# ibejarano/Pynama

Hardware: AMD Instinct MI355X
Metric: assembled element-DOFs/sec + CG iterations/sec, 10M-DOF Poisson, 1/2/4/8 MI355X (higher is better)
Workload: dtype f64

## Files before the change

include/pynama_hip.h:

```cpp
#ifndef PYNAMA_HIP_H
#define PYNAMA_HIP_H

#include <stdint.h>

#ifdef __cplusplus
extern "C" {
#endif

typedef struct pyn_ctx pyn_ctx;

enum {
  PYN_OK = 0,
  PYN_EINVAL = -1,
  PYN_EHIP = -2,
  PYN_ENCCL = -3,
  PYN_ENOTCONV = -4,
  PYN_ENOGPU = -5
};

enum { PYN_Q_FULL = 0, PYN_Q_RED = 1, PYN_Q_NODAL = 2 };

enum {
  PYN_FORM_LAPLACE = 0,
  PYN_FORM_MASS_NODAL = 1,
// ... 81 lines not shown
int pyn_vec_maxpy(pyn_ctx* ctx, int y, int x, int m, const int* ids, const double* w);
int pyn_ts_step_finish(pyn_ctx* ctx, int x, int m, const int* ids, const double* hb, const double* hd, double atol, double rtol,
                       double* wnorm);

int pyn_nodeset_create(pyn_ctx* ctx, int64_t n, const int32_t* nodes, int* set_id);
int pyn_nodeset_destroy(pyn_ctx* ctx, int set_id);
enum {
  PYN_FIELD_TG2D_VEL = 0, PYN_FIELD_TG2D_VORT = 1,
  PYN_FIELD_TG3D_VEL = 2, PYN_FIELD_TG3D_VORT = 3, PYN_FIELD_TG3D_CONV = 4, PYN_FIELD_TG3D_DIFF = 5,
  PYN_FIELD_SEN2D_VEL = 6, PYN_FIELD_SEN2D_VORT = 7, PYN_FIELD_SEN2D_CONV = 8, PYN_FIELD_SEN2D_DIFF = 9,
  PYN_FIELD_COUNT = 10
};
#define PYN_FIELD_MAX_PARAMS 4
int pyn_field_info(int field, int* dim, int* bs, int* nparams);
int pyn_field_eval(pyn_ctx* ctx, int field, const double* params, int nparams, int set_id, int vec_id);
int pyn_vec_set_nodes(pyn_ctx* ctx, int vec_id, int set_id, const double* values, int nvalues, const uint8_t* dofs);

int pyn_assemble_kle(pyn_ctx* ctx, double alpha_d, double alpha_w, int K, int Krhs, int Rw, int Rd,
                     int variant);
int pyn_assemble_kle_noslip(pyn_ctx* ctx, double alpha_d, double alpha_w, const int* mat_ids);
int pyn_assemble_scalar(pyn_ctx* ctx, int form, int A, int Arhs, int variant);
int pyn_elem_local(pyn_ctx* ctx, int form, double alpha_d, double alpha_w, const double* corners,
                   double* out0, double* out1, double* out2);

int pyn_assemble_operator(pyn_ctx* ctx, int rule, int nterms, const int32_t* terms, const double* coef, int mat_id);
int pyn_elem_operator_local(pyn_ctx* ctx, int rule, int br, int bc, int nterms, const int32_t* terms,
                            const double* coef, const double* corners, double* out);

int pyn_spmv(pyn_ctx* ctx, int mat_id, int x_vec, int y_vec);
int pyn_product_last(pyn_ctx* ctx, int64_t* info);
int pyn_product_choose(int br, int bc, int npat, int maxw, int64_t nnzb, int64_t n_owned, int rhs_compact, int solver, int image,
                       int sell_image, int block_sell, int no_csrlb, int no_sell, double bcsr_min_avg, int bcsr_lanes, int bcsr_unroll,
                       int* kind, int* W, int* lanes, int* unroll);
int pyn_assemble_last(pyn_ctx* ctx, int64_t* info);
int pyn_assemble_choose(const int64_t* request, const int64_t* facts, const int64_t* knobs, int64_t* out);
int pyn_assemble_choose_layout(char* buf, int len);
enum { PYN_MATFREE_OFF = 0, PYN_MATFREE_LAPLACE = 1, PYN_MATFREE_KLE = 2, PYN_MATFREE_KLE_GENERAL = 3,
       PYN_MATFREE_KLE_NGL3_GENERAL = 4 };
int pyn_matfree_set(pyn_ctx* ctx, int op, double alpha_d, double alpha_w);
int pyn_matfree_apply(pyn_ctx* ctx, int op, int x_vec, int y_vec);
typedef struct pyn_solve_opts {
  int method;
  int pc;
  int norm_type;
  int maxit;
  int restart;
  int fixed_iters;
  int profile;
  int cg_variant;
  int gmres_orthog;
  int matfree;
  double rtol, atol, dtol;
} pyn_solve_opts;
typedef struct pyn_solve_info {
  int iters;
  int reason;
  double rnorm;
  double rnorm0;
  double true_resid;
  double solve_ms;
  double spmv_ms;
  int spmv_launches;
  double reduce_ms;
  double halo_ms;
} pyn_solve_info;
int pyn_solve(pyn_ctx* ctx, int mat_id, int b_vec, int x_vec, const pyn_solve_opts* opts,
// ... 35 lines not shown
```

pynama_amd/_lib.py:

```python
from __future__ import annotations

import ctypes as C
import os
import subprocess
import sys

import numpy as np

_HERE = os.path.dirname(os.path.abspath(__file__))
LIB_PATH = os.environ.get("PYNAMA_LIB_PATH") or os.path.join(_HERE, "libpynama_hip.so")
CSRC = os.path.join(_HERE, "csrc")

Q_FULL, Q_RED, Q_NODAL = 0, 1, 2
FORM_LAPLACE, FORM_MASS_NODAL, FORM_MASS_FULL, FORM_KLE, FORM_OPERATOR = 0, 1, 2, 3, 4
KSP_CG, KSP_GMRES = 0, 1
MATFREE_OFF, MATFREE_LAPLACE, MATFREE_KLE, MATFREE_KLE_GENERAL, MATFREE_KLE_NGL3_GENERAL = 0, 1, 2, 3, 4
PC_NONE, PC_JACOBI, PC_MG = 0, 1, 2
MG_MAX_LEVELS = 16
TS_MAX_STAGES = 8
NORM_PRECONDITIONED, NORM_UNPRECONDITIONED, NORM_NATURAL = 0, 1, 2
T_SYMBOLIC, T_ASSEMBLE, T_SPMV, T_SOLVE = 0, 1, 2, 3
(FIELD_TG2D_VEL, FIELD_TG2D_VORT, FIELD_TG3D_VEL, FIELD_TG3D_VORT, FIELD_TG3D_CONV, FIELD_TG3D_DIFF,
 FIELD_SEN2D_VEL, FIELD_SEN2D_VORT, FIELD_SEN2D_CONV, FIELD_SEN2D_DIFF) = range(10)
FIELD_COUNT, FIELD_MAX_PARAMS = 10, 4
# ... 66 lines not shown
    "pyn_mat_get_values": [_P, _I, _pf64],
    "pyn_mat_get_diagonal": [_P, _I, _I],
    "pyn_mat_axpy": [_P, _I, _D, _I],
    "pyn_mat_row_scale": [_P, _I, _I],
    "pyn_vec_create": [_P, _I, C.POINTER(_I)],
    "pyn_vec_destroy": [_P, _I],
    "pyn_vec_set_host": [_P, _I, _pf64],
    "pyn_vec_set_local_host": [_P, _I, _pf64],
    "pyn_vec_get_host": [_P, _I, _pf64],
    "pyn_vec_fill": [_P, _I, _D],
    "pyn_vec_scatter_host": [_P, _I, _L, _pi32, _pf64, _I],
    "pyn_vec_axpby": [_P, _I, _D, _I, _D, _I],
    "pyn_vec_pointwise_mult": [_P, _I, _I, _I],
    "pyn_vec_reciprocal": [_P, _I],
    "pyn_vec_vtensv": [_P, _I, _I],
    "pyn_vec_dot": [_P, _I, _I, C.POINTER(_D)],
    "pyn_vec_norm": [_P, _I, _I, C.POINTER(_D)],
    "pyn_vec_maxpy": [_P, _I, _I, _I, _pi32, _pf64],
    "pyn_ts_step_finish": [_P, _I, _I, _pi32, _pf64, _P, _D, _D, C.POINTER(_D)],
    "pyn_nodeset_create": [_P, _L, _P, C.POINTER(_I)],
    "pyn_nodeset_destroy": [_P, _I],
    "pyn_field_info": [_I, C.POINTER(_I), C.POINTER(_I), C.POINTER(_I)],
    "pyn_field_eval": [_P, _I, _pf64, _I, _I, _I],
    "pyn_vec_set_nodes": [_P, _I, _I, _pf64, _I, _P],
    "pyn_assemble_kle": [_P, _D, _D, _I, _I, _I, _I, _I],
    "pyn_assemble_kle_noslip": [_P, _D, _D, C.POINTER(_I)],
    "pyn_assemble_scalar": [_P, _I, _I, _I, _I],
    "pyn_elem_local": [_P, _I, _D, _D, _pf64, _P, _P, _P],
    "pyn_assemble_operator": [_P, _I, _I, _pi32, _pf64, _I],
    "pyn_elem_operator_local": [_P, _I, _I, _I, _I, _pi32, _pf64, _pf64, _pf64],
    "pyn_spmv": [_P, _I, _I, _I],
    "pyn_product_last": [_P, _pi64],
    "pyn_product_choose": [_I] * 4 + [_L, _L] + [_I] * 7 + [_D, _I, _I] + [C.POINTER(_I)] * 4,
    "pyn_assemble_last": [_P, _pi64],
    "pyn_assemble_choose": [_pi64, _pi64, _pi64, _pi64],
    "pyn_assemble_choose_layout": [C.c_char_p, _I],
    "pyn_matfree_apply": [_P, _I, _I, _I],
    "pyn_matfree_set": [_P, _I, _D, _D],
    "pyn_solve": [_P, _I, _I, _I, C.POINTER(SolveOpts), C.POINTER(SolveInfo)],
    "pyn_direct_max_rows": [],
    "pyn_solve_direct": [_P, _I, _I, _I, C.POINTER(SolveInfo)],
    "pyn_direct_band_info": [_P, _I, C.POINTER(_L), C.POINTER(_L), C.POINTER(_L)],
    "pyn_solve_direct_band": [_P, _I, _I, _I, _L, C.POINTER(SolveInfo)],
    "pyn_mg_setup": [_P, _I, C.POINTER(MgOpts)],
    "pyn_mg_info": [_P, _I, C.POINTER(_I), _pi64, _pf64, C.POINTER(_D), C.POINTER(_I)],
    "pyn_mg_apply": [_P, _I, _I, _I],
    "pyn_mg_level_get": [_P, _I, _I, _pf64],
    "pyn_ibm_set": [_P, _I, _I, _L, _pf64, _pf64, _pf64, _pf64],
    "pyn_ibm_interp": [_P, _I, _pf64],
    "pyn_ibm_spread": [_P, _pf64, _I],
    "pyn_ibm_correct": [_P, _I, _pf64, _pf64],
    "pyn_ibm_matrix_get": [_P, _pf64],
    "pyn_ibm_info": [_P, _pi64],
    "pyn_ibm_clear": [_P],
    "pyn_timers_get": [_P, _pf64, _I],
}

_lib = None


def build_library(force=False):
    if force:
        subprocess.check_call(["make", "-C", CSRC, "clean"])
    subprocess.check_call(["make", "-C", CSRC, "-j4"])
    return LIB_PATH

# ... 46 lines not shown

def ho_tables_1d(ngl):
    n = int(ngl)
    if n < 2:
        raise PynamaHipError(f"ho_tables_1d: ngl {n} out of range")
    t = dict(xl=np.zeros(n), wl=np.zeros(n), Dl=np.zeros((n, n)), xr=np.zeros(n - 1), wr=np.zeros(n - 1),
             Br=np.zeros((n - 1, n)), Gr=np.zeros((n - 1, n)))
    _check(load_library().pyn_ho_tables_1d(n, *(t[k] for k in ("xl", "wl", "Dl", "xr", "wr", "Br", "Gr"))))
    return t


def ho_local_lattice(ngl, dim):
    loc = np.zeros((int(ngl) ** int(dim), int(dim)), np.int32)
    _check(load_library().pyn_ho_local_lattice(int(ngl), int(dim), loc))
    return loc


def field_info(field):
    d, b, n = _I(0), _I(0), _I(0)
    _check(load_library().pyn_field_info(int(field), C.byref(d), C.byref(b), C.byref(n)))
    return d.value, b.value, n.value


def product_choose(br, bc, npat, maxw, nnzb, n_owned, rhs_compact=False, solver=False, image=False, sell_image=False,
                   block_sell=False, no_csrlb=False, no_sell=False, bcsr_min_avg=None, bcsr_lanes=None, bcsr_unroll=None):
    out = [_I(0) for _ in range(4)]
    _check(load_library().pyn_product_choose(
        int(br), int(bc), int(npat), int(maxw), int(nnzb), int(n_owned), int(rhs_compact), int(solver), int(image), int(sell_image),
        int(block_sell), int(no_csrlb), int(no_sell), -1.0 if bcsr_min_avg is None else float(bcsr_min_avg),
        -1 if bcsr_lanes is None else int(bcsr_lanes), -1 if bcsr_unroll is None else int(bcsr_unroll), *(C.byref(o) for o in out)))
    return tuple(o.value for o in out)


ASSEMBLY_KINDS = ("none", "generic", "p1", "patch", "lattice", "march", "kle_lattice", "rowrun")
AK_NONE, AK_GENERIC, AK_P1, AK_PATCH, AK_LATTICE, AK_MARCH, AK_KLE_LATTICE, AK_ROWRUN = range(8)
_ASM_LAST_KEYS = ("kind", "shape", "k_closed", "rw_closed", "generic", "krhs_completed", "dinv", "count")


def assemble_choose_layout():
    buf = C.create_string_buffer(4096)
    _check(load_library().pyn_assemble_choose_layout(buf, len(buf)))
    return {part.split(":")[0]: tuple(n for n in part.split(":")[1].split(",") if n) for part in buf.value.decode().split(";")}


def assemble_choose(request, facts, knobs=None):
    layout = assemble_choose_layout()
    given = {"request": dict({"variant": 1}, **request), "facts": dict(facts), "knobs": dict(knobs or {})}
    arrays = {}
    for part, names in layout.items():
        unknown = set(given[part]) - set(names)
        if unknown:
            raise PynamaHipError(f"assemble_choose: unknown {part} {sorted(unknown)}")
        arrays[part] = np.array([int(given[part].get(n, -1 if part == "knobs" else 0)) for n in names], np.int64)
    out = np.zeros(8, np.int64)
    _check(load_library().pyn_assemble_choose(arrays["request"], arrays["facts"], arrays["knobs"], out))
    return dict({k: int(v) for k, v in zip(_ASM_LAST_KEYS[:7], out)}, rowrun_candidate=int(out[7]))


class _stdout_to_stderr:

    def __enter__(self):
        sys.stdout.flush()
        self._saved = os.dup(1)
        os.dup2(2, 1)

    def __exit__(self, *exc):
# ... 489 lines not shown
```

pynama_amd/csrc/pyn_internal.h:

```cpp
#pragma once
#include <hip/hip_runtime.h>
#include <rccl/rccl.h>

#include <algorithm>
#include <atomic>
#include <cstdint>
#include <cstdio>
#include <functional>
#include <map>
#include <memory>
#include <string>
#include <type_traits>
#include <utility>
#include <vector>

#include "../../include/pynama_hip.h"

void pyn_set_error(const char* fmt, ...);

#define PYN_HIP(call)                                                                         \
  do {                                                                                        \
    hipError_t e_ = (call);                                                                   \
    if (e_ != hipSuccess) {                                                                   \
      pyn_set_error("%s:%d %s -> %s", __FILE__, __LINE__, #call, hipGetErrorString(e_));      \
// ... 68 lines not shown
  T* get() const { return p_; }
  operator T*() const { return p_; }
};
template <typename T>
using DevBuf = Buf<T, false>;
template <typename T>
using PinBuf = Buf<T, true>;

struct DevTmp : DevBuf<unsigned char> {
  template <typename T>
  T* as() const {
    return reinterpret_cast<T*>(get());
  }
};

template <typename T>
inline int dev_upload(DevBuf<T>& dst, const T* src, size_t n, hipStream_t s) {
  PYN_HIP(dst.alloc(n));
  if (n && src) PYN_HIP(hipMemcpyAsync(dst.get(), src, n * sizeof(T), hipMemcpyHostToDevice, s));
  return PYN_OK;
}

struct QuadTab {
  int ngp = 0;
  DevBuf<double> w;
  DevBuf<double> H;
  DevBuf<double> Hrs;
  DevBuf<double> HrsCoo;
  double wsum = 0.0;
  bool const_grad = false;
};

enum ProductKind { PK_NONE = 0, PK_RAW = 1, PK_SELL = 2, PK_SELLP = 3, PK_SELLB_X = 4, PK_SELLB_D = 5, PK_CSRL = 6, PK_CSRLB = 7, PK_BCSR = 8 };
struct ProductPlan {
  ProductKind kind = PK_NONE;
  int W = 0;
  int lg = 0, unroll = 0;
  size_t lds = 0;
  int wg_cap = -1;
  int max_grid = INT32_MAX;
};

struct MgHier;
struct IbmState;
struct MgHierDelete { void operator()(MgHier* h) const; };
struct IbmStateDelete { void operator()(IbmState* s) const; };

struct DMat {
  int br = 0, bc = 0;
  DevBuf<double> val;
  DevBuf<double> sell_val;
  bool sell_valid = false;
  ProductPlan plan;
  DevBuf<double> dinv;
  bool dinv_valid = false;
  DevBuf<double> lu;
  DevBuf<int> lu_piv;
  int64_t lu_n = 0;
  bool lu_valid = false;
  DevBuf<double> band;
  DevBuf<int> band_perm;
  int64_t band_n = 0, band_kl = 0, band_ku = 0;
  bool band_valid = false;
  std::unique_ptr<MgHier, MgHierDelete> mg;
  bool mg_valid = false;
  int64_t rhs_clean = -2;
  bool rhs_compact = false;
  int64_t c_stamp = -1;
  int64_t c_nr = 0, c_nnzb = 0;
  DevBuf<int32_t> c_crow;
  DevBuf<int32_t> c_rsel;
  DevBuf<int32_t> c_cptr;
  bool live = false;
// ... 397 lines not shown
```

pynama_amd/csrc/pyn_sell.hip:

```cpp
#include <hipcub/hipcub.hpp>

#include "pyn_internal.h"

namespace {

constexpr int PAT_MAX = 256;
constexpr int PAT_W = 32;

constexpr int SH = 64;

__global__ void sell_width_kernel(const int32_t* __restrict__ rowptr, int64_t n_rows, int br, int bc, int64_t n_slices,
                                  int* __restrict__ w) {
  for (int64_t s = (int64_t)blockIdx.x * blockDim.x + threadIdx.x; s < n_slices; s += (int64_t)gridDim.x * blockDim.x) {
    int64_t r0 = s * SH, r1 = r0 + SH < n_rows ? r0 + SH : n_rows;
    int m = 0;
    for (int64_t r = r0; r < r1; ++r) {
      const int64_t i = r / br;
      m = max(m, (rowptr[i + 1] - rowptr[i]) * bc);
    }
    w[s] = m;
  }
}

template <bool WITH_COLS>
// ... 188 lines not shown
  for (int64_t r = (int64_t)blockIdx.x * blockDim.x + threadIdx.x; r < n_rows; r += (int64_t)gridDim.x * blockDim.x) {
    const unsigned long long x = h[r];
    int l = 0, hgh = nu;
    while (l < hgh) {
      int m = (l + hgh) >> 1;
      if (uniq[m] < x)
        l = m + 1;
      else
        hgh = m;
    }
    pid[r] = l;
    rep[l] = (int32_t)r;
  }
}

__global__ void pat_table_kernel(const int32_t* __restrict__ rowptr, const int32_t* __restrict__ colidx,
                                 const int32_t* __restrict__ rep, int nu, int32_t* __restrict__ tab, int32_t* __restrict__ tlen) {
  const int p = blockIdx.x;
  if (p >= nu) return;
  const int r = rep[p];
  const int lo = rowptr[r], len = rowptr[r + 1] - lo;
  if (threadIdx.x == 0) tlen[p] = len;
  for (int k = threadIdx.x; k < PAT_W; k += blockDim.x) tab[p * PAT_W + k] = k < len ? colidx[lo + k] - r : 0;
}

__global__ void pat_verify_kernel(const int32_t* __restrict__ rowptr, const int32_t* __restrict__ colidx, int64_t n_rows,
                                  const int32_t* __restrict__ pid, const int32_t* __restrict__ tab,
                                  const int32_t* __restrict__ tlen, int* __restrict__ bad) {
  for (int64_t r = (int64_t)blockIdx.x * blockDim.x + threadIdx.x; r < n_rows; r += (int64_t)gridDim.x * blockDim.x) {
    const int lo = rowptr[r], len = rowptr[r + 1] - lo;
    const int p = pid[r];
    bool ok = len == tlen[p];
    for (int k = 0; ok && k < len; ++k) ok = colidx[lo + k] == (int32_t)r + tab[p * PAT_W + k];
    if (!ok) *bad = 1;
  }
}

template <bool DOT>
__global__ void __launch_bounds__(256) sellp_spmv_kernel(const int64_t* __restrict__ sptr, const int* __restrict__ sw,
                                                         const int32_t* __restrict__ pid, const int32_t* __restrict__ tab,
                                                         int npat, const double* __restrict__ sval,
                                                         const double* __restrict__ x, double* __restrict__ y, int64_t n_rows,
                                                         int64_t n_slices, const int* __restrict__ flag,
                                                         double* __restrict__ part, int64_t s_begin, int part_off, int64_t hole_begin, int64_t hole_len) {
  extern __shared__ int32_t ltab[];
  __shared__ double smd[4];
  if (flag && flag[0]) return;
  for (int i = threadIdx.x; i < (npat + 1) * PAT_W; i += 256) ltab[i] = i < npat * PAT_W ? tab[i] : 0;
  __syncthreads();
  const int lane = threadIdx.x & 63;
  const int64_t w0 = ((int64_t)blockIdx.x * blockDim.x + threadIdx.x) >> 6;
  const int64_t nw = ((int64_t)gridDim.x * blockDim.x) >> 6;
  double dot = 0.0;
  for (int64_t sq = s_begin + w0; sq < n_slices; sq += nw) {
    const int64_t s = sq >= hole_begin ? sq + hole_len : sq;
    const int64_t row = s * SH + lane;
    const int wd = sw[s];
    const double* __restrict__ v = sval + sptr[s] + lane;
    const int32_t* __restrict__ t = ltab + (row < n_rows ? pid[row] : npat) * PAT_W;
    const int64_t rb = row < n_rows ? row : 0;
    double a0 = 0.0, a1 = 0.0, a2 = 0.0, a3 = 0.0;
    int k = 0;
    for (; k + 4 <= wd; k += 4) {
      const double v0 = v[(k + 0) * SH], v1 = v[(k + 1) * SH], v2 = v[(k + 2) * SH], v3 = v[(k + 3) * SH];
      a0 = fma(v0, x[rb + t[k + 0]], a0);
      a1 = fma(v1, x[rb + t[k + 1]], a1);
      a2 = fma(v2, x[rb + t[k + 2]], a2);
      a3 = fma(v3, x[rb + t[k + 3]], a3);
    }
    for (; k < wd; ++k) a0 = fma(v[k * SH], x[rb + t[k]], a0);
    const double acc = (a0 + a1) + (a2 + a3);
    if (row < n_rows) {
      y[row] = acc;
      if (DOT) dot += acc * x[row];
    }
  }
  if (DOT) {
    dot = wsum64(dot);
    if (lane == 0) smd[threadIdx.x >> 6] = dot;
    __syncthreads();
    if (threadIdx.x == 0) part[part_off + blockIdx.x] = smd[0] + smd[1] + smd[2] + smd[3];
  }
}

template <typename T_>
__device__ __forceinline__ T_ ld_stream(const T_* p) {
  return __builtin_nontemporal_load(p);
}

constexpr int CSRL_WAVES = 4;
template <int W, bool DOT>
__global__ void __launch_bounds__(64 * CSRL_WAVES) csrl_spmv_kernel(const int32_t* __restrict__ rowptr, const int32_t* __restrict__ pid,
                                                                    const int32_t* __restrict__ tab, int npat, const double* __restrict__ val,
                                                                    const double* __restrict__ x, double* __restrict__ y, int64_t n_rows,
                                                                    int64_t n_slices, const int* __restrict__ flag, double* __restrict__ part,
                                                                    int64_t s_begin, int part_off, int64_t hole_begin, int64_t hole_len) {
  extern __shared__ double csrl_lds[];
  __shared__ double smd[CSRL_WAVES];
  if (flag && flag[0]) return;
  int32_t* ltab = reinterpret_cast<int32_t*>(csrl_lds + CSRL_WAVES * 64 * W);
  for (int i = threadIdx.x; i < (npat + 1) * PAT_W; i += 64 * CSRL_WAVES) ltab[i] = i < npat * PAT_W ? tab[i] : 0;
  __syncthreads();
  const int lane = threadIdx.x & 63, wv = threadIdx.x >> 6;
  double* __restrict__ buf = csrl_lds + wv * 64 * W;
  const int64_t w0 = (int64_t)blockIdx.x * CSRL_WAVES + wv;
  const int64_t nw = (int64_t)gridDim.x * CSRL_WAVES;
  double dot = 0.0;
  int nrp0 = 0, nrp1 = 0;
  {
    const int64_t sq = s_begin + w0;
    if (sq < n_slices) {
      const int64_t r = (sq >= hole_begin ? sq + hole_len : sq) * SH + lane;
      nrp0 = rowptr[r < n_rows ? r : n_rows];
      nrp1 = rowptr[r < n_rows ? r + 1 : n_rows];
    }
  }
  for (int64_t sq = s_begin + w0; sq < n_slices; sq += nw) {
    const int64_t s = sq >= hole_begin ? sq + hole_len : sq;
    const int64_t row = s * SH + lane;
    const bool live = row < n_rows;
    const int rp0 = nrp0, rp1 = nrp1;
    if (sq + nw < n_slices) {
      const int64_t r = ((sq + nw) >= hole_begin ? sq + nw + hole_len : sq + nw) * SH + lane;
      nrp0 = rowptr[r < n_rows ? r : n_rows];
      nrp1 = rowptr[r < n_rows ? r + 1 : n_rows];
    }
    const int base = __builtin_amdgcn_readfirstlane(rp0);
    const int total = __builtin_amdgcn_readlane(rp1, 63) - base;
    const int off = rp0 - base, len = rp1 - rp0;
    const double* __restrict__ v = val + base;
    double vr[W];
#pragma unroll
    for (int j = 0; j < W; ++j) vr[j] = (64 * j + lane < total) ? ld_stream(v + 64 * j + lane) : 0.0;
    const int32_t* __restrict__ t = ltab + (live ? pid[row] : npat) * PAT_W;
    const int64_t rb = live ? row : 0;
    double xg[W];
#pragma unroll
    for (int k = 0; k < W; ++k) xg[k] = x[rb + (k < len ? t[k] : 0)];
#pragma unroll
    for (int j = 0; j < W; ++j) buf[64 * j + lane] = vr[j];
    __builtin_amdgcn_fence(__ATOMIC_RELEASE, "wavefront");
    __builtin_amdgcn_wave_barrier();
    __builtin_amdgcn_fence(__ATOMIC_ACQUIRE, "wavefront");
    double a0 = 0.0, a1 = 0.0;
#pragma unroll
    for (int k = 0; k + 1 < W; k += 2) {
      a0 = fma(k < len ? buf[off + k] : 0.0, xg[k], a0);
      a1 = fma(k + 1 < len ? buf[off + k + 1] : 0.0, xg[k + 1], a1);
    }
    if (W & 1) a0 = fma(W - 1 < len ? buf[off + W - 1] : 0.0, xg[W - 1], a0);
    const double acc = a0 + a1;
    if (live) {
      y[row] = acc;
      if (DOT) dot += acc * x[row];
    }
    __builtin_amdgcn_fence(__ATOMIC_RELEASE, "wavefront");
    __builtin_amdgcn_wave_barrier();
  }
  if (DOT) {
    dot = wsum64(dot);
    if (lane == 0) smd[wv] = dot;
    __syncthreads();
    if (threadIdx.x == 0) {
      double sm = 0.0;
      for (int i = 0; i < CSRL_WAVES; ++i) sm += smd[i];
      part[part_off + blockIdx.x] = sm;
    }
  }
}

constexpr int CSRLB_WAVES = 2;
template <int W, int BR, int BC, bool GL, bool DOT>
__global__ void __launch_bounds__(64 * CSRLB_WAVES) csrlb_spmv_kernel(const int32_t* __restrict__ rowptr, const int32_t* __restrict__ pid,
                                                                      const int32_t* __restrict__ tab, int npat, const double* __restrict__ val,
                                                                      const double* __restrict__ x, double* __restrict__ y, int64_t n_rows,
                                                                      int64_t n_slices, const int* __restrict__ flag, double* __restrict__ part,
                                                                      int64_t s_begin, int part_off, int64_t hole_begin, int64_t hole_len) {
  extern __shared__ double csrl_lds[];
  __shared__ double smd[CSRLB_WAVES];
  if (flag && flag[0]) return;
  int32_t* ltab = reinterpret_cast<int32_t*>(csrl_lds + CSRLB_WAVES * 64 * W);
  for (int i = threadIdx.x; i < (npat + 1) * PAT_W; i += 64 * CSRLB_WAVES) ltab[i] = i < npat * PAT_W ? tab[i] : 0;
  __syncthreads();
  const int lane = threadIdx.x & 63, wv = threadIdx.x >> 6;
  double* __restrict__ buf = csrl_lds + wv * 64 * W;
  const int64_t w0 = (int64_t)blockIdx.x * CSRLB_WAVES + wv;
  const int64_t nw = (int64_t)gridDim.x * CSRLB_WAVES;
  const int64_t n_nodes = n_rows / BR;
  double dot = 0.0;
  for (int64_t sq = s_begin + w0; sq < n_slices; sq += nw) {
// ... 258 lines not shown
  if (DOT) block_partial(dot, part);
}

}

namespace {
__device__ __forceinline__ int lat_axis_class(int ngl, int c, int N) {
  if (ngl == 2) return c == 0 ? 0 : (c == N - 1 ? 2 : 1);
  if (c & 1) return 3;
  return c == 0 ? 0 : (c == N - 1 ? 2 : 1);
}
__global__ void pat_lattice_pid_kernel(int ngl, int dim, int NX, int NY, int NZ, int64_t n_rows, int32_t* __restrict__ pid) {
  const int64_t i = (int64_t)blockIdx.x * blockDim.x + threadIdx.x;
  if (i >= n_rows) return;
  const int ncls = ngl == 2 ? 3 : 4;
  const int x = (int)(i % NX), y = (int)((i / NX) % NY), z = (int)(i / ((int64_t)NX * NY));
  int id = lat_axis_class(ngl, y, NY) * ncls + lat_axis_class(ngl, x, NX);
  if (dim == 3) id += lat_axis_class(ngl, z, NZ) * ncls * ncls;
  pid[i] = id;
}
__global__ void pat_verify_sample_kernel(const int32_t* __restrict__ rowptr, const int32_t* __restrict__ colidx, int64_t n_rows, int64_t stride,
                                         const int32_t* __restrict__ pid, const int32_t* __restrict__ tab, const int32_t* __restrict__ tlen,
                                         int* __restrict__ bad) {
  const int64_t t = (int64_t)blockIdx.x * blockDim.x + threadIdx.x;
  int64_t r = t * stride;
  if (r >= n_rows) {
    if (r - stride >= n_rows || t == 0) return;
    r = n_rows - 1;
  }
  const int lo = rowptr[r], len = rowptr[r + 1] - lo;
  const int p = pid[r];
  bool ok = len == tlen[p];
  for (int k = 0; ok && k < len; ++k) ok = colidx[lo + k] == (int32_t)r + tab[p * PAT_W + k];
  if (!ok) *bad = 1;
}
}

static int lattice_pattern_dictionary(pyn_ctx* c, bool* done) {
  *done = false;
  if (getenv("PYNAMA_NO_LATTICE_PATTERNS")) return PYN_OK;
  const BoxLattice& B = c->box;
  if (!(c->lat.valid || c->ho3.valid) || (B.ngl == 3 && B.dim == 3) || c->n_ghost != 0 || !B.natural()) return PYN_OK;
  const int ngl = B.ngl, dim = B.dim, NX = B.NX, NY = B.ny(), NZ = B.nz();
  const int ncls = ngl == 2 ? 3 : 4;
  const int npat = dim == 3 ? ncls * ncls * ncls : ncls * ncls;
  auto axis_offs = [&](int cls, int* out) {
    int lo, hi;
    if (ngl == 2) {
      lo = cls == 0 ? 0 : -1;
      hi = cls == 2 ? 0 : 1;
    } else if (cls == 3) {
      lo = -1;
      hi = 1;
    } else {
      lo = cls == 0 ? 0 : -2;
      hi = cls == 2 ? 0 : 2;
    }
    int n = 0;
    for (int d = lo; d <= hi; ++d) out[n++] = d;
    return n;
  };
  std::vector<int32_t> tab((size_t)PAT_MAX * PAT_W, 0), tlen((size_t)PAT_MAX, 0);
  for (int p = 0; p < npat; ++p) {
    const int cx = p % ncls, cy = (p / ncls) % ncls, cz = p / (ncls * ncls);
    int ox[5], oy[5], oz[5] = {0, 0, 0, 0, 0};
    const int nxo = axis_offs(cx, ox), nyo = axis_offs(cy, oy), nzo = dim == 3 ? axis_offs(cz, oz) : 1;
// ... 73 lines not shown
  PYN_HIP(hipMemsetAsync(ptab, 0, (size_t)PAT_MAX * PAT_W * sizeof(int32_t), s));
  pat_assign_kernel<<<grid, 256, 0, s>>>(h, n, hu, (int)nu, pid, t_rep.as<int32_t>());
  pat_table_kernel<<<(int)nu, 64, 0, s>>>(c->d_rowptr, c->d_colidx, t_rep.as<int32_t>(), (int)nu, ptab, t_len.as<int32_t>());
  pat_verify_kernel<<<grid, 256, 0, s>>>(c->d_rowptr, c->d_colidx, n, pid, ptab, t_len.as<int32_t>(), t_bad.as<int>());
  int hbad = 0;
  PYN_HIP(hipMemcpyAsync(&hbad, t_bad.get(), sizeof(int), hipMemcpyDeviceToHost, s));
  PYN_HIP(hipStreamSynchronize(s));
  if (hbad != 0) return PYN_OK;
  c->sell_pid = std::move(pid);
  c->sell_tab = std::move(ptab);
  c->sell_npat = (int)nu;
  return PYN_OK;
}

__global__ void slice_ghost_flag_kernel(const int32_t* __restrict__ rowptr, const int32_t* __restrict__ colidx, int64_t n_owned,
                                        int br, int64_t ns, int* __restrict__ flags) {
  for (int64_t s = (int64_t)blockIdx.x * blockDim.x + threadIdx.x; s < ns; s += (int64_t)gridDim.x * blockDim.x) {
    const int64_t r0 = s * SH, r1 = std::min<int64_t>(r0 + SH, n_owned * br) - 1;
    int f = 0;
    for (int64_t i = r0 / br; i <= r1 / br; ++i) f |= colidx[rowptr[i + 1] - 1] >= n_owned;
    flags[s] = f;
  }
}

struct ProductFacts {
  int br, bc, npat, maxw;
  int64_t nnzb, n_owned;
  bool rhs_compact, solver, image;
};
struct ProductKnobs {
  bool sell_image, block_sell, no_csrlb, no_sell;
  double bcsr_min_avg;
  int bcsr_lanes, bcsr_unroll, bcsr_wgs, csrlb_wgs, csr_wgs, max_grid;
};
static int env_int(const char* name) {
  const char* e = getenv(name);
  return e ? std::max(0, atoi(e)) : -1;
}
static ProductKnobs read_knobs() {
  const char* avg = getenv("PYNAMA_BCSR_MIN_AVG");
  return {getenv("PYNAMA_SELL_IMAGE") != nullptr, getenv("PYNAMA_BLOCK_SELL") != nullptr, getenv("PYNAMA_NO_CSRLB") != nullptr,
          getenv("PYNAMA_NO_SELL") != nullptr, avg ? atof(avg) : 128.0, env_int("PYNAMA_BCSR_LANES"), env_int("PYNAMA_BCSR_UNROLL"),
          env_int("PYNAMA_BCSR_WGS_PER_CU"), env_int("PYNAMA_CSRLB_WGS_PER_CU"), env_int("PYNAMA_CSR_SPMV_WGS_PER_CU"),
          env_int("PYNAMA_SPMV_MAX_GRID")};
}

static bool sell_shape(int bc) { return bc == 1 || bc == 2 || bc == 3 || bc == 6; }
static bool bcsr_shape(int br, int bc) {
  return (br == bc && (br == 1 || br == 2 || br == 3)) || (bc == 1 && (br == 2 || br == 3)) || (br == 1 && (bc == 2 || bc == 3)) ||
         (br == 3 && bc == 2) || (br == 2 && bc == 3) || (br == 6 && bc == 3) || (br == 3 && bc == 6);
}
static bool raw_only(const ProductFacts& f, const ProductKnobs& k) { return !f.rhs_compact && (k.no_sell || !sell_shape(f.bc)); }

static ProductPlan product_choose(const ProductFacts& f, const ProductKnobs& k, bool* keep_image) {
  auto pick = [&](ProductPlan p, bool keep) { *keep_image = keep; return p; };
  const double avg = (double)f.nnzb * f.bc / (double)std::max<int64_t>(1, f.n_owned);
  auto bcsr = [&](bool keep) {
    const int g = k.bcsr_lanes, lg = g >= 0 ? (g >= 64 ? 6 : g >= 32 ? 5 : g >= 16 ? 4 : 3) : (avg >= 56.0 ? 4 : 3);
    const int u = k.bcsr_unroll >= 0 ? k.bcsr_unroll : (avg >= 24.0 ? 8 : 4);
    return pick({PK_BCSR, 0, lg, (u == 2 || u == 3 || u == 8) ? u : 4}, keep);
  };
  const bool scalar = f.br == 1 && f.bc == 1;
  if (f.rhs_compact) return bcsr_shape(f.br, f.bc) ? bcsr(true) : pick({}, true);
  if (raw_only(f, k)) return pick({PK_RAW}, true);
  if (scalar && f.npat > 0 && f.maxw <= PAT_W && !k.sell_image) return pick({PK_CSRL, f.maxw <= 27 ? 27 : 32}, false);
  if (f.br == 2 && f.bc == 2 && f.npat > 0 && f.maxw <= 50 && !k.block_sell && !k.no_csrlb)
    return pick({PK_CSRLB, f.maxw <= 18 ? 18 : (f.maxw <= 32 ? 32 : 50)}, false);
  int bm = (k.block_sell || !bcsr_shape(f.br, f.bc)) ? 0 : (avg >= k.bcsr_min_avg ? 1 : 2);
  if (scalar && !(f.maxw > PAT_W && !k.sell_image)) bm = 0;
  if (bm == 1) return bcsr(false);
  if (bm == 2 && !f.solver && !f.image) return bcsr(true);
  return pick({scalar ? (f.npat > 0 ? PK_SELLP : PK_SELL) : (f.npat > 0 ? PK_SELLB_D : PK_SELLB_X)}, true);
}

extern "C" int pyn_product_choose(int br, int bc, int npat, int maxw, int64_t nnzb, int64_t n_owned, int rhs_compact, int solver,
                                  int image, int sell_image, int block_sell, int no_csrlb, int no_sell, double bcsr_min_avg,
                                  int bcsr_lanes, int bcsr_unroll, int* kind, int* W, int* lanes, int* unroll) {
  PYN_CHECK(kind && W && lanes && unroll, "pyn_product_choose: NULL output");
  PYN_CHECK(br > 0 && bc > 0 && npat >= 0 && maxw >= 0 && nnzb >= 0 && n_owned >= 0, "pyn_product_choose: bad argument");
  const ProductKnobs k{sell_image != 0, block_sell != 0, no_csrlb != 0, no_sell != 0, bcsr_min_avg >= 0.0 ? bcsr_min_avg : 128.0,
                       std::max(-1, bcsr_lanes), std::max(-1, bcsr_unroll), -1, -1, -1, -1};
  bool keep_image;
  const ProductPlan ch = product_choose({br, bc, npat, maxw, nnzb, n_owned, rhs_compact != 0, solver != 0, image != 0}, k, &keep_image);
  *kind = ch.kind;
  *W = ch.W;
  *lanes = ch.kind == PK_BCSR ? 1 << ch.lg : 0;
  *unroll = ch.unroll;
  return PYN_OK;
}

static int sell_structure(pyn_ctx* c, const DMat& A, SellShape** out) {
  hipStream_t s = c->stream;
  const int64_t n = c->n_owned * A.br;
  const int64_t ns = (n + SH - 1) / SH;
  if (!c->sell_dict_built) {
    std::vector<int32_t> rp((size_t)c->n_owned + 1);
    PYN_HIP(hipMemcpyAsync(rp.data(), c->d_rowptr, (c->n_owned + 1) * sizeof(int32_t), hipMemcpyDeviceToHost, s));
    PYN_HIP(hipStreamSynchronize(s));
    int maxlen = 0;
    for (int64_t i = 0; i < c->n_owned; ++i) maxlen = std::max(maxlen, rp[i + 1] - rp[i]);
    PYN_TRY(build_pattern_dictionary(c, maxlen));
    c->sell_dict_built = true;
  }
  *out = const_cast<SellShape*>(pyn_sell_shape(c, A));
  if (*out) return PYN_OK;
  SellShape q;
  q.br = A.br;
  q.bc = A.bc;
  q.ns = ns;
  PYN_HIP(q.w.alloc(ns));
  sell_width_kernel<<<(int)std::min<int64_t>((ns + 255) / 256, 4096), 256, 0, s>>>(c->d_rowptr, n, A.br, A.bc, ns, q.w);
  std::vector<int> w((size_t)ns);
  PYN_HIP(hipMemcpyAsync(w.data(), q.w, ns * sizeof(int), hipMemcpyDeviceToHost, s));
  PYN_HIP(hipStreamSynchronize(s));
  std::vector<int64_t> ptr((size_t)ns + 1);
  ptr[0] = 0;
  for (int64_t i = 0; i < ns; ++i) {
    ptr[i + 1] = ptr[i] + (int64_t)w[i] * SH;
    q.maxw = std::max(q.maxw, w[i]);
  }
  q.total = ptr[ns];
// ... 118 lines not shown
  spmv_kernel<32, DOT><<<*grid, 256, 0, L.st>>>(L.c->d_rowptr, L.c->d_colidx, L.A.val, L.x, L.y, rows, L.A.br, L.A.bc, L.flag, L.part);
  return PYN_OK;
}

template <bool DOT>
int launch_sell(const Launch& L, int grid) {
  pyn_ctx* c = L.c;
  const SellShape& S = *L.S;
  if (L.P.kind == PK_SELLP)
    sellp_spmv_kernel<DOT><<<grid, 256, L.P.lds, L.st>>>(S.ptr, S.w, c->sell_pid, c->sell_tab, c->sell_npat, L.A.sell_val, L.x, L.y, c->n_owned,
                                                         L.s1, L.flag, L.part, L.s0, L.poff, L.hb, L.hl);
  else
    sell_spmv_kernel<DOT><<<grid, 256, 0, L.st>>>(S.ptr, S.w, S.col, L.A.sell_val, L.x, L.y, c->n_owned, L.s1, L.flag, L.part, L.s0, L.poff, L.hb,
                                                  L.hl);
  return PYN_OK;
}

template <int BC, bool DOT>
int launch_sellb(const Launch& L, int grid) {
  pyn_ctx* c = L.c;
  const SellShape& S = *L.S;
  const int64_t n = c->n_owned * L.A.br;
  if (L.P.kind == PK_SELLB_D)
    sellb_spmv_kernel<BC, true, DOT><<<grid, 256, L.P.lds, L.st>>>(S.ptr, S.w, c->sell_pid, c->sell_tab, c->sell_npat, nullptr, L.A.sell_val, L.x,
                                                                   L.y, n, L.A.br, L.s1, L.flag, L.part, L.s0, L.poff, L.hb, L.hl);
  else
    sellb_spmv_kernel<BC, false, DOT><<<grid, 256, 0, L.st>>>(S.ptr, S.w, nullptr, nullptr, 0, S.col, L.A.sell_val, L.x, L.y, n, L.A.br, L.s1,
                                                              L.flag, L.part, L.s0, L.poff, L.hb, L.hl);
  return PYN_OK;
}

template <int W, bool DOT>
int launch_csrl(const Launch& L, int* grid) {
  static bool attr = false;
  if (!attr) {
    PYN_HIP(hipFuncSetAttribute(reinterpret_cast<const void*>(csrl_spmv_kernel<W, DOT>), hipFuncAttributeMaxDynamicSharedMemorySize,
                                (int)(CSRL_WAVES * 64 * W * sizeof(double) + (PAT_MAX + 1) * PAT_W * sizeof(int32_t))));
    attr = true;
  }
  pyn_ctx* c = L.c;
  *grid = persistent_grid(L, (L.s1 - L.s0 + CSRL_WAVES - 1) / CSRL_WAVES, 0);
  PYN_CHECK(L.poff + *grid <= PYN_MAX_PARTIALS, "partial buffer overflow");
  csrl_spmv_kernel<W, DOT><<<*grid, 64 * CSRL_WAVES, L.P.lds, L.st>>>(c->d_rowptr, c->sell_pid, c->sell_tab, c->sell_npat, L.A.val, L.x, L.y,
                                                                      c->n_owned, L.s1, L.flag, L.part, L.s0, L.poff, L.hb, L.hl);
  return PYN_OK;
}

template <int W, bool DOT>
int launch_csrlb(const Launch& L, int* grid) {
  constexpr bool GL = W > 32;
  static int per_cu = 0;
  if (!per_cu) {
    PYN_HIP(hipFuncSetAttribute(reinterpret_cast<const void*>(csrlb_spmv_kernel<W, 2, 2, GL, DOT>), hipFuncAttributeMaxDynamicSharedMemorySize,
                                (int)(CSRLB_WAVES * 64 * W * sizeof(double) + (PAT_MAX + 1) * PAT_W * sizeof(int32_t))));
    PYN_HIP(hipOccupancyMaxActiveBlocksPerMultiprocessor(&per_cu, csrlb_spmv_kernel<W, 2, 2, GL, DOT>, 64 * CSRLB_WAVES, L.P.lds));
    per_cu = std::max(1, per_cu);
  }
  pyn_ctx* c = L.c;
  *grid = persistent_grid(L, (L.s1 - L.s0 + CSRLB_WAVES - 1) / CSRLB_WAVES, 256 * per_cu);
  PYN_CHECK(L.poff + *grid <= PYN_MAX_PARTIALS, "partial buffer overflow");
  csrlb_spmv_kernel<W, 2, 2, GL, DOT><<<*grid, 64 * CSRLB_WAVES, L.P.lds, L.st>>>(c->d_rowptr, c->sell_pid, c->sell_tab, c->sell_npat, L.A.val,
                                                                                  L.x, L.y, c->n_owned * L.A.br, L.s1, L.flag, L.part, L.s0,
                                                                                  L.poff, L.hb, L.hl);
  return PYN_OK;
}

template <int BR, int BC, int U, bool DOT>
int launch_bcsr_u(const Launch& L, int* grid) {
  static int per_cu = 0;
  if (!per_cu) {
    PYN_HIP(hipOccupancyMaxActiveBlocksPerMultiprocessor(&per_cu, bcsr_spmv_kernel<BR, BC, U, DOT>, 256, 0));
    per_cu = std::max(1, std::min(per_cu, 8));
  }
  pyn_ctx* c = L.c;
  const int npw = 64 >> L.P.lg;
  *grid = persistent_grid(L, (L.s1 - L.s0 + 4 * npw - 1) / (4 * npw), 256 * per_cu);
  PYN_CHECK(L.poff + *grid <= PYN_MAX_PARTIALS, "partial buffer overflow");
// ... 107 lines not shown
```

Before: 197.0 billion.

## Add software-pipelined CSRL SpMV kernel that prefetches next slice metadata and values

Adds a new CSRL SpMV kernel that software-pipelines each wave's persistent loop. Row metadata is fetched two slices ahead, and the next slice's values and x-gather are issued while the current slice is multiplied from LDS. It uses launch bounds with two blocks per CU and vectorised int4 reads of the pattern table. The old kernel stays available via PYNAMA_CSRL_PLAIN. The pattern validator now also requires zero padding in table entries past each row's length, since the new gather reads all W offsets. The risk is higher register pressure and the hand-written waitcnt and fence sequencing.

```diff
diff --git a/include/pynama_hip.h b/include/pynama_hip.h
--- a/include/pynama_hip.h
+++ b/include/pynama_hip.h
@@ -137,6 +137,9 @@
 int pyn_product_choose(int br, int bc, int npat, int maxw, int64_t nnzb, int64_t n_owned, int rhs_compact, int solver, int image,
                        int sell_image, int block_sell, int no_csrlb, int no_sell, double bcsr_min_avg, int bcsr_lanes, int bcsr_unroll,
                        int* kind, int* W, int* lanes, int* unroll);
+int pyn_product_choose_loop(int br, int bc, int npat, int maxw, int64_t nnzb, int64_t n_owned, int rhs_compact, int solver, int image,
+                            int sell_image, int block_sell, int no_csrlb, int no_sell, double bcsr_min_avg, int bcsr_lanes,
+                            int bcsr_unroll, int csrl_plain, int* kind, int* W, int* lanes, int* unroll, int* loop);
 int pyn_assemble_last(pyn_ctx* ctx, int64_t* info);
 int pyn_assemble_choose(const int64_t* request, const int64_t* facts, const int64_t* knobs, int64_t* out);
 int pyn_assemble_choose_layout(char* buf, int len);
diff --git a/pynama_amd/_lib.py b/pynama_amd/_lib.py
--- a/pynama_amd/_lib.py
+++ b/pynama_amd/_lib.py
@@ -122,6 +122,7 @@
     "pyn_spmv": [_P, _I, _I, _I],
     "pyn_product_last": [_P, _pi64],
     "pyn_product_choose": [_I] * 4 + [_L, _L] + [_I] * 7 + [_D, _I, _I] + [C.POINTER(_I)] * 4,
+    "pyn_product_choose_loop": [_I] * 4 + [_L, _L] + [_I] * 7 + [_D, _I, _I, _I] + [C.POINTER(_I)] * 5,
     "pyn_assemble_last": [_P, _pi64],
     "pyn_assemble_choose": [_pi64, _pi64, _pi64, _pi64],
     "pyn_assemble_choose_layout": [C.c_char_p, _I],
@@ -234,6 +235,18 @@
     return tuple(o.value for o in out)
 
 
+def product_choose_loop(br, bc, npat, maxw, nnzb, n_owned, csrl_plain=False, rhs_compact=False, solver=False, image=False,
+                        sell_image=False, block_sell=False, no_csrlb=False, no_sell=False, bcsr_min_avg=None, bcsr_lanes=None,
+                        bcsr_unroll=None):
+    out = [_I(0) for _ in range(5)]
+    _check(load_library().pyn_product_choose_loop(
+        int(br), int(bc), int(npat), int(maxw), int(nnzb), int(n_owned), int(rhs_compact), int(solver), int(image), int(sell_image),
+        int(block_sell), int(no_csrlb), int(no_sell), -1.0 if bcsr_min_avg is None else float(bcsr_min_avg),
+        -1 if bcsr_lanes is None else int(bcsr_lanes), -1 if bcsr_unroll is None else int(bcsr_unroll), int(csrl_plain),
+        *(C.byref(o) for o in out)))
+    return tuple(o.value for o in out)
+
+
 ASSEMBLY_KINDS = ("none", "generic", "p1", "patch", "lattice", "march", "kle_lattice", "rowrun")
 AK_NONE, AK_GENERIC, AK_P1, AK_PATCH, AK_LATTICE, AK_MARCH, AK_KLE_LATTICE, AK_ROWRUN = range(8)
 _ASM_LAST_KEYS = ("kind", "shape", "k_closed", "rw_closed", "generic", "krhs_completed", "dinv", "count")
diff --git a/pynama_amd/csrc/pyn_internal.h b/pynama_amd/csrc/pyn_internal.h
--- a/pynama_amd/csrc/pyn_internal.h
+++ b/pynama_amd/csrc/pyn_internal.h
@@ -124,6 +124,7 @@
 };
 
 enum ProductKind { PK_NONE = 0, PK_RAW = 1, PK_SELL = 2, PK_SELLP = 3, PK_SELLB_X = 4, PK_SELLB_D = 5, PK_CSRL = 6, PK_CSRLB = 7, PK_BCSR = 8 };
+enum { CSRL_LOOP_PIPELINED = 0, CSRL_LOOP_PLAIN = 1 };
 struct ProductPlan {
   ProductKind kind = PK_NONE;
   int W = 0;
@@ -131,6 +132,7 @@
   size_t lds = 0;
   int wg_cap = -1;
   int max_grid = INT32_MAX;
+  int loop = 0;
 };
 
 struct MgHier;
diff --git a/pynama_amd/csrc/pyn_sell.hip b/pynama_amd/csrc/pyn_sell.hip
--- a/pynama_amd/csrc/pyn_sell.hip
+++ b/pynama_amd/csrc/pyn_sell.hip
@@ -244,6 +244,7 @@
     const int p = pid[r];
     bool ok = len == tlen[p];
     for (int k = 0; ok && k < len; ++k) ok = colidx[lo + k] == (int32_t)r + tab[p * PAT_W + k];
+    for (int k = len; ok && k < PAT_W; ++k) ok = tab[p * PAT_W + k] == 0;
     if (!ok) *bad = 1;
   }
 }
@@ -302,11 +303,11 @@
 
 constexpr int CSRL_WAVES = 4;
 template <int W, bool DOT>
-__global__ void __launch_bounds__(64 * CSRL_WAVES) csrl_spmv_kernel(const int32_t* __restrict__ rowptr, const int32_t* __restrict__ pid,
-                                                                    const int32_t* __restrict__ tab, int npat, const double* __restrict__ val,
-                                                                    const double* __restrict__ x, double* __restrict__ y, int64_t n_rows,
-                                                                    int64_t n_slices, const int* __restrict__ flag, double* __restrict__ part,
-                                                                    int64_t s_begin, int part_off, int64_t hole_begin, int64_t hole_len) {
+__global__ void __launch_bounds__(64 * CSRL_WAVES) csrl_plain_spmv_kernel(const int32_t* __restrict__ rowptr, const int32_t* __restrict__ pid,
+                                                                          const int32_t* __restrict__ tab, int npat, const double* __restrict__ val,
+                                                                          const double* __restrict__ x, double* __restrict__ y, int64_t n_rows,
+                                                                          int64_t n_slices, const int* __restrict__ flag, double* __restrict__ part,
+                                                                          int64_t s_begin, int part_off, int64_t hole_begin, int64_t hole_len) {
   extern __shared__ double csrl_lds[];
   __shared__ double smd[CSRL_WAVES];
   if (flag && flag[0]) return;
@@ -368,6 +369,122 @@
     }
     __builtin_amdgcn_fence(__ATOMIC_RELEASE, "wavefront");
     __builtin_amdgcn_wave_barrier();
+  }
+  if (DOT) {
+    dot = wsum64(dot);
+    if (lane == 0) smd[wv] = dot;
+    __syncthreads();
+    if (threadIdx.x == 0) {
+      double sm = 0.0;
+      for (int i = 0; i < CSRL_WAVES; ++i) sm += smd[i];
+      part[part_off + blockIdx.x] = sm;
+    }
+  }
+}
+
+template <int W, bool DOT>
+__global__ void __launch_bounds__(64 * CSRL_WAVES, 2) csrl_spmv_kernel(const int32_t* __restrict__ rowptr, const int32_t* __restrict__ pid,
+                                                                       const int32_t* __restrict__ tab, int npat, const double* __restrict__ val,
+                                                                       const double* __restrict__ x, double* __restrict__ y, int64_t n_rows,
+                                                                       int64_t n_slices, const int* __restrict__ flag, double* __restrict__ part,
+                                                                       int64_t s_begin, int part_off, int64_t hole_begin, int64_t hole_len) {
+  extern __shared__ __attribute__((aligned(16))) double csrl_pipe_lds[];
+  __shared__ double smd[CSRL_WAVES];
+  if (flag && flag[0]) return;
+  int32_t* ltab = reinterpret_cast<int32_t*>(csrl_pipe_lds + CSRL_WAVES * 64 * W);
+  for (int i = threadIdx.x; i < (npat + 1) * PAT_W; i += 64 * CSRL_WAVES) ltab[i] = i < npat * PAT_W ? tab[i] : 0;
+  __syncthreads();
+  const int lane = threadIdx.x & 63, wv = __builtin_amdgcn_readfirstlane(threadIdx.x >> 6);
+  double* __restrict__ buf = csrl_pipe_lds + wv * 64 * W;
+  const int64_t nw = (int64_t)gridDim.x * CSRL_WAVES;
+  double dot = 0.0;
+  int64_t sq = s_begin + (int64_t)blockIdx.x * CSRL_WAVES + wv;
+  if (sq < n_slices) {
+    struct Slice {
+      int total, off, len, p;
+      int64_t row;
+      bool live;
+    };
+    double vr[W], xg[W], xd = 0.0;
+    struct Meta {
+      int rp0, rp1, pid;
+    };
+    Meta m1, m2;
+    auto meta = [&](int64_t q) {
+      q = q < n_slices ? q : n_slices - 1;
+      const int64_t r = (q >= hole_begin ? q + hole_len : q) * SH + lane;
+      const bool lv = r < n_rows;
+      return Meta{rowptr[lv ? r : n_rows], rowptr[lv ? r + 1 : n_rows], pid[lv ? r : n_rows - 1]};
+    };
+    auto start = [&](int64_t q, Slice& S) {
+      S.row = (q >= hole_begin ? q + hole_len : q) * SH + lane;
+      S.live = S.row < n_rows;
+      S.p = S.live ? m1.pid : npat;
+      const int base = __builtin_amdgcn_readfirstlane(m1.rp0);
+      S.total = __builtin_amdgcn_readlane(m1.rp1, 63) - base;
+      S.off = m1.rp0 - base;
+      S.len = m1.rp1 - m1.rp0;
+      const double* __restrict__ v = val + (S.total > 0 ? base : 0);
+      const int last = (S.total > 0 ? S.total : 1) - 1;
+#pragma unroll
+      for (int j = 0; j < W; ++j) vr[j] = ld_stream(v + min(64 * j + lane, last));
+    };
+    auto gather = [&](const Slice& S) {
+      const int4* __restrict__ t4 = reinterpret_cast<const int4*>(ltab + S.p * PAT_W);
+      int tk[4 * ((W + 3) / 4)];
+#pragma unroll
+      for (int q = 0; q < (W + 3) / 4; ++q) {
+        const int4 t = t4[q];
+        tk[4 * q] = t.x, tk[4 * q + 1] = t.y, tk[4 * q + 2] = t.z, tk[4 * q + 3] = t.w;
+      }
+      __builtin_amdgcn_s_waitcnt(0xC07F);
+      const int64_t rb = S.live ? S.row : 0;
+#pragma unroll
+      for (int k = 0; k < W; ++k) xg[k] = x[rb + tk[k]];
+      if (DOT) xd = x[rb];
+    };
+    auto park = [&](const Slice& S) {
+#pragma unroll
+      for (int j = 0; j < W; ++j) buf[64 * j + lane] = (64 * j + lane < S.total) ? vr[j] : 0.0;
+    };
+    auto multiply = [&](const Slice& S) {
+      __builtin_amdgcn_fence(__ATOMIC_RELEASE, "wavefront");
+      __builtin_amdgcn_wave_barrier();
+      __builtin_amdgcn_fence(__ATOMIC_ACQUIRE, "wavefront");
+      const int off = S.off, len = S.len;
+      double a0 = 0.0, a1 = 0.0;
+#pragma unroll
+      for (int k = 0; k + 1 < W; k += 2) {
+        a0 = fma(k < len ? buf[off + k] : 0.0, xg[k], a0);
+        a1 = fma(k + 1 < len ? buf[off + k + 1] : 0.0, xg[k + 1], a1);
+      }
+      if (W & 1) a0 = fma(W - 1 < len ? buf[off + W - 1] : 0.0, xg[W - 1], a0);
+      const double acc = a0 + a1;
+      if (S.live) {
+        y[S.row] = acc;
+        if (DOT) dot += acc * xd;
+      }
+      __builtin_amdgcn_fence(__ATOMIC_RELEASE, "wavefront");
+      __builtin_amdgcn_wave_barrier();
+    };
+    Slice S, Sn;
+    m1 = meta(sq);
+    start(sq, S);
+    m1 = meta(sq + nw);
+    m2 = meta(sq + 2 * nw);
+    gather(S);
+    for (; sq + nw < n_slices; sq += nw) {
+      park(S);
+      multiply(S);
+      start(sq + nw, Sn);
+      m1 = m2;
+      asm volatile("" : "+v"(m1.rp0), "+v"(m1.rp1), "+v"(m1.pid));
+      m2 = meta(sq + 3 * nw);
+      gather(Sn);
+      S = Sn;
+    }
+    park(S);
+    multiply(S);
   }
   if (DOT) {
     dot = wsum64(dot);
@@ -692,6 +809,7 @@
   const int p = pid[r];
   bool ok = len == tlen[p];
   for (int k = 0; ok && k < len; ++k) ok = colidx[lo + k] == (int32_t)r + tab[p * PAT_W + k];
+  for (int k = len; ok && k < PAT_W; ++k) ok = tab[p * PAT_W + k] == 0;
   if (!ok) *bad = 1;
 }
 }
@@ -831,6 +949,7 @@
   bool sell_image, block_sell, no_csrlb, no_sell;
   double bcsr_min_avg;
   int bcsr_lanes, bcsr_unroll, bcsr_wgs, csrlb_wgs, csr_wgs, max_grid;
+  bool csrl_plain;
 };
 static int env_int(const char* name) {
   const char* e = getenv(name);
@@ -841,7 +960,8 @@
   return {getenv("PYNAMA_SELL_IMAGE") != nullptr, getenv("PYNAMA_BLOCK_SELL") != nullptr, getenv("PYNAMA_NO_CSRLB") != nullptr,
           getenv("PYNAMA_NO_SELL") != nullptr, avg ? atof(avg) : 128.0, env_int("PYNAMA_BCSR_LANES"), env_int("PYNAMA_BCSR_UNROLL"),
           env_int("PYNAMA_BCSR_WGS_PER_CU"), env_int("PYNAMA_CSRLB_WGS_PER_CU"), env_int("PYNAMA_CSR_SPMV_WGS_PER_CU"),
-          env_int("PYNAMA_SPMV_MAX_GRID")};
+          env_int("PYNAMA_SPMV_MAX_GRID"),
+          getenv("PYNAMA_CSRL_PLAIN") != nullptr};
 }
 
 static bool sell_shape(int bc) { return bc == 1 || bc == 2 || bc == 3 || bc == 6; }
@@ -862,7 +982,11 @@
   const bool scalar = f.br == 1 && f.bc == 1;
   if (f.rhs_compact) return bcsr_shape(f.br, f.bc) ? bcsr(true) : pick({}, true);
   if (raw_only(f, k)) return pick({PK_RAW}, true);
-  if (scalar && f.npat > 0 && f.maxw <= PAT_W && !k.sell_image) return pick({PK_CSRL, f.maxw <= 27 ? 27 : 32}, false);
+  if (scalar && f.npat > 0 && f.maxw <= PAT_W && !k.sell_image) {
+    ProductPlan p{PK_CSRL, f.maxw <= 27 ? 27 : 32};
+    p.loop = (k.csrl_plain || f.nnzb == 0) ? CSRL_LOOP_PLAIN : CSRL_LOOP_PIPELINED;
+    return pick(p, false);
+  }
   if (f.br == 2 && f.bc == 2 && f.npat > 0 && f.maxw <= 50 && !k.block_sell && !k.no_csrlb)
     return pick({PK_CSRLB, f.maxw <= 18 ? 18 : (f.maxw <= 32 ? 32 : 50)}, false);
   int bm = (k.block_sell || !bcsr_shape(f.br, f.bc)) ? 0 : (avg >= k.bcsr_min_avg ? 1 : 2);
@@ -872,20 +996,30 @@
   return pick({scalar ? (f.npat > 0 ? PK_SELLP : PK_SELL) : (f.npat > 0 ? PK_SELLB_D : PK_SELLB_X)}, true);
 }
 
-extern "C" int pyn_product_choose(int br, int bc, int npat, int maxw, int64_t nnzb, int64_t n_owned, int rhs_compact, int solver,
-                                  int image, int sell_image, int block_sell, int no_csrlb, int no_sell, double bcsr_min_avg,
-                                  int bcsr_lanes, int bcsr_unroll, int* kind, int* W, int* lanes, int* unroll) {
-  PYN_CHECK(kind && W && lanes && unroll, "pyn_product_choose: NULL output");
+extern "C" int pyn_product_choose_loop(int br, int bc, int npat, int maxw, int64_t nnzb, int64_t n_owned, int rhs_compact, int solver,
+                                       int image, int sell_image, int block_sell, int no_csrlb, int no_sell, double bcsr_min_avg,
+                                       int bcsr_lanes, int bcsr_unroll, int csrl_plain, int* kind, int* W, int* lanes, int* unroll,
+                                       int* loop) {
+  PYN_CHECK(kind && W && lanes && unroll && loop, "pyn_product_choose: NULL output");
   PYN_CHECK(br > 0 && bc > 0 && npat >= 0 && maxw >= 0 && nnzb >= 0 && n_owned >= 0, "pyn_product_choose: bad argument");
   const ProductKnobs k{sell_image != 0, block_sell != 0, no_csrlb != 0, no_sell != 0, bcsr_min_avg >= 0.0 ? bcsr_min_avg : 128.0,
-                       std::max(-1, bcsr_lanes), std::max(-1, bcsr_unroll), -1, -1, -1, -1};
+                       std::max(-1, bcsr_lanes), std::max(-1, bcsr_unroll), -1, -1, -1, -1, csrl_plain != 0};
   bool keep_image;
   const ProductPlan ch = product_choose({br, bc, npat, maxw, nnzb, n_owned, rhs_compact != 0, solver != 0, image != 0}, k, &keep_image);
   *kind = ch.kind;
   *W = ch.W;
   *lanes = ch.kind == PK_BCSR ? 1 << ch.lg : 0;
   *unroll = ch.unroll;
+  *loop = ch.loop;
   return PYN_OK;
+}
+
+extern "C" int pyn_product_choose(int br, int bc, int npat, int maxw, int64_t nnzb, int64_t n_owned, int rhs_compact, int solver,
+                                  int image, int sell_image, int block_sell, int no_csrlb, int no_sell, double bcsr_min_avg,
+                                  int bcsr_lanes, int bcsr_unroll, int* kind, int* W, int* lanes, int* unroll) {
+  int loop;
+  return pyn_product_choose_loop(br, bc, npat, maxw, nnzb, n_owned, rhs_compact, solver, image, sell_image, block_sell, no_csrlb, no_sell,
+                                 bcsr_min_avg, bcsr_lanes, bcsr_unroll, 0, kind, W, lanes, unroll, &loop);
 }
 
 static int sell_structure(pyn_ctx* c, const DMat& A, SellShape** out) {
@@ -1070,17 +1204,13 @@
 
 template <int W, bool DOT>
 int launch_csrl(const Launch& L, int* grid) {
-  static bool attr = false;
-  if (!attr) {
-    PYN_HIP(hipFuncSetAttribute(reinterpret_cast<const void*>(csrl_spmv_kernel<W, DOT>), hipFuncAttributeMaxDynamicSharedMemorySize,
-                                (int)(CSRL_WAVES * 64 * W * sizeof(double) + (PAT_MAX + 1) * PAT_W * sizeof(int32_t))));
-    attr = true;
-  }
   pyn_ctx* c = L.c;
+  auto kern = L.P.loop == CSRL_LOOP_PLAIN ? csrl_plain_spmv_kernel<W, DOT> : csrl_spmv_kernel<W, DOT>;
+  PYN_TRY(pyn_kernel_lds(c, kern, CSRL_WAVES * 64 * W * sizeof(double) + (PAT_MAX + 1) * PAT_W * sizeof(int32_t)));
   *grid = persistent_grid(L, (L.s1 - L.s0 + CSRL_WAVES - 1) / CSRL_WAVES, 0);
   PYN_CHECK(L.poff + *grid <= PYN_MAX_PARTIALS, "partial buffer overflow");
-  csrl_spmv_kernel<W, DOT><<<*grid, 64 * CSRL_WAVES, L.P.lds, L.st>>>(c->d_rowptr, c->sell_pid, c->sell_tab, c->sell_npat, L.A.val, L.x, L.y,
-                                                                      c->n_owned, L.s1, L.flag, L.part, L.s0, L.poff, L.hb, L.hl);
+  kern<<<*grid, 64 * CSRL_WAVES, L.P.lds, L.st>>>(c->d_rowptr, c->sell_pid, c->sell_tab, c->sell_npat, L.A.val, L.x, L.y, c->n_owned, L.s1,
+                                                  L.flag, L.part, L.s0, L.poff, L.hb, L.hl);
   return PYN_OK;
 }
 
```

After: 196.7 billion. No clear change (-0.1%).
